# TaWeiTu/vp8

Measured on NVIDIA B200. Metric: decoded 1080p frames/s, higher is better.
Workload: dtype u8

## Files before the change

vp8_b200/csrc/cuda/recon_kernels.cu:

```cuda
#include "recon_kernels.h"

#include <algorithm>
#include <cstring>

namespace vp8r {

__constant__ int c_taps[2][8][2];
__constant__ int c_taps6[2][8][6];
__constant__ unsigned short c_bpred_lut[10 * 16];

static int PackTaps(int a, int b, int c, int d) {
  return (a & 0xff) | ((b & 0xff) << 8) | ((c & 0xff) << 16) | ((d & 0xff) << 24);
}

static void BuildBpredLut(unsigned short *lut) {
  auto L = [](int k) { return 3 - k; };
  auto A = [](int k) { return 5 + k; };
  const int P = 4;
  auto put3 = [&](int mode, int y, int x, int a, int b, int c) {
    lut[mode * 16 + y * 4 + x] = (unsigned short)(a | (b << 4) | (c << 8) | (0 << 12));
  };
  auto put2 = [&](int mode, int y, int x, int a, int c) {
    lut[mode * 16 + y * 4 + x] = (unsigned short)(a | (a << 4) | (c << 8) | (1 << 12));
  };
// ... 347 lines not shown
      out1 = AddResidual4(out1, rb.x, rb.y);
    }
    uint8_t *d = job.cur.y + (ptrdiff_t)(mb_r * 16 + y0) * job.pitch_y + mb_c * 16 + 4 * w;
    *reinterpret_cast<unsigned *>(d) = out0;
    *reinterpret_cast<unsigned *>(d + job.pitch_y) = out1;
  }
  {
    const int pl = lane >> 4, y = (lane >> 1) & 7, w = lane & 1;
    const unsigned *h = s.hc[pl];
    unsigned out;
    if (cfr) {
      unsigned e[6], o[6];
#pragma unroll
      for (int k = 0; k < 6; ++k) {
        const unsigned r = h[(y + k) * 2 + w];
        e[k] = __byte_perm(r, 0, 0x4240);
        o[k] = __byte_perm(r, 0, 0x4341);
      }
      out = Vert6(e, o, c_taps6[bil][cfr]);
    } else if (cfc == 0) {
      const int dx2 = ((g.cwx + kBorder) & 15) + 2;
      const unsigned *p = reinterpret_cast<const unsigned *>((pl ? tile->cv : tile->cu) + (y + 2) * kTmaChromaBoxW) + (dx2 >> 2) + w;
      out = __funnelshift_r(p[0], p[1], (dx2 & 3) * 8);
    } else {
      out = h[(y + 2) * 2 + w];
    }
    if (has_res) {
      const uint2 ra = *reinterpret_cast<const uint2 *>(&s.res[16 + pl * 4 + (y >> 2) * 2 + w][(y & 3) * 4]);
      out = AddResidual4(out, ra.x, ra.y);
    }
    uint8_t *d = (pl ? job.cur.v : job.cur.u) + (ptrdiff_t)(mb_r * 8 + y) * job.pitch_c + mb_c * 8 + 4 * w;
    *reinterpret_cast<unsigned *>(d) = out;
  }
}

constexpr int kInterWarps = 4;
constexpr int kInterMinBlocks = 14;

__device__ __forceinline__ void InterOneMacroblock(const DevFrameJob &job, int mb_r, int mb_c, int lane, InterScratch &scratch, InterTile *tile) {
  const int mb_index = mb_r * job.mb_cols + mb_c;
  vp8r_mb_info mb;
  {
    const int4 *p = reinterpret_cast<const int4 *>(job.mbs + mb_index);
    int4 a = __ldg(p), b = __ldg(p + 1);
    mb.flags = a.x; mb.coef_mask = a.y; mb.coef_offset = a.z;
    mb.mv[0] = (short)(a.w & 0xffff); mb.mv[1] = (short)(a.w >> 16);
    mb.aux[0] = b.x; mb.aux[1] = b.y;
  }
  if (!(mb.flags & VP8R_MB_IS_INTER)) return;

  const bool split = ((mb.flags >> VP8R_MB_MODE_SHIFT) & 7) == 4;
  WholeMbGeometry geo{};
  if (!split) {
    geo = WholeGeometry(job, mb, mb_r, mb_c);
    if (lane == 0) {
      const DevTensorMap *maps = job.ref_tmap[(mb.flags >> VP8R_MB_REF_SHIFT) & 3];
      MbarExpectTx(&tile->bar, kInterTileTxBytes);
      TmaLoad2D(tile->luma, maps + 0, (geo.wx + kBorder) & ~15, geo.wy + kBorder, &tile->bar);
      TmaLoad2D(tile->cu, maps + 1, (geo.cwx + kBorder) & ~15, geo.cwy + kBorder, &tile->bar);
      TmaLoad2D(tile->cv, maps + 2, (geo.cwx + kBorder) & ~15, geo.cwy + kBorder, &tile->bar);
    }
  }
  const bool has_res = mb.coef_mask != 0;
  if (has_res) WarpResidual(job, mb, lane, scratch);
  if (!split) {
    InterMacroblockWhole(job, mb_r, mb_c, lane, scratch, has_res, geo, tile);
    return;
  }
  __syncwarp();
  if (lane >= 24) return;

  const int ref_id = (mb.flags >> VP8R_MB_REF_SHIFT) & 3;
  const int *split_mv = reinterpret_cast<const int *>(job.payload + (size_t)mb.aux[0] * 16);

  int mvr, mvc, bx, by, pitch, plane_w, plane_h;
  const uint8_t *ref;
  uint8_t *dst;
  if (lane < 16) {
    const int m = __ldg(split_mv + lane);
    mvr = (short)(m & 0xffff);
    mvc = m >> 16;
    by = mb_r * 16 + (lane >> 2) * 4;
    bx = mb_c * 16 + (lane & 3) * 4;
    pitch = job.pitch_y;
    plane_w = job.mb_cols * 16;
    plane_h = job.mb_rows * 16;
    ref = job.ref[ref_id].y;
    dst = job.cur.y;
  } else {
    const int b = lane & 3, i = b >> 1, j = b & 1;
    const int k0 = i * 8 + j * 2;
    const int m0 = __ldg(split_mv + k0), m1 = __ldg(split_mv + k0 + 1), m2 = __ldg(split_mv + k0 + 4),
              m3 = __ldg(split_mv + k0 + 5);
    const int sr = s16((short)(m0 & 0xffff) + (short)(m1 & 0xffff) + (short)(m2 & 0xffff) + (short)(m3 & 0xffff));
    const int sc = s16((m0 >> 16) + (m1 >> 16) + (m2 >> 16) + (m3 >> 16));
    mvr = (sr >= 0 ? (sr + 4) : (sr - 4)) / 8;
    mvc = (sc >= 0 ? (sc + 4) : (sc - 4)) / 8;
    if (job.version == 3) {
      mvr &= ~7;
      mvc &= ~7;
    }
    by = mb_r * 8 + i * 4;
    bx = mb_c * 8 + j * 4;
    pitch = job.pitch_c;
    plane_w = job.mb_cols * 8;
    plane_h = job.mb_rows * 8;
    ref = lane < 20 ? job.ref[ref_id].u : job.ref[ref_id].v;
    dst = lane < 20 ? job.cur.u : job.cur.v;
  }

  const int fr = mvr & 7, fc = mvc & 7;
  int wy = by + (mvr >> 3) - 2, wx = bx + (mvc >> 3) - 2;
  wy = min(max(wy, -kBorder), plane_h + kBorder - 9);
  wx = min(max(wx, -kBorder), plane_w + kBorder - 9);
  const uint8_t *__restrict__ wp = ref + (ptrdiff_t)wy * pitch + wx;
  const uint2 *__restrict__ wrow = reinterpret_cast<const uint2 *>(wp - ((size_t)wp & 7));
  const bool upper = ((size_t)wp & 4) != 0;
  const unsigned shift = ((unsigned)(size_t)wp & 3u) * 8;
  const int wpitch = pitch >> 3;

  const int bil = job.version != 0;
  const int r_lo = fr ? 0 : 2, r_hi = fr ? 9 : 6;
  const int t03 = c_taps[bil][fc][0], t45 = c_taps[bil][fc][1];
  const TapsAt ta = MakeTapsAt(t03, t45);
  unsigned h[9];
#pragma unroll
  for (int i = 0; i < 9; ++i) {
    if (i >= r_lo && i < r_hi) {
      const uint2 a = __ldg(wrow + i * wpitch), b = __ldg(wrow + i * wpitch + 1);
      const unsigned w0 = upper ? a.y : a.x, w1 = upper ? b.x : a.y, w2 = upper ? b.y : b.x;
      const unsigned lo = __funnelshift_r(w0, w1, shift), mid = __funnelshift_r(w1, w2, shift), hi = w2 >> shift;
      h[i] = fc ? Filter4T(lo, mid, hi, t03, t45, ta) : __funnelshift_r(lo, mid, 16);
    }
  }
  unsigned out[4];
  if (fr) {
    const int v03 = c_taps[bil][fr][0], v45 = c_taps[bil][fr][1];
    const int t[6] = {(signed char)v03, (signed char)(v03 >> 8), (signed char)(v03 >> 16), v03 >> 24,
                      (signed char)v45, (signed char)(v45 >> 8)};
    unsigned e[9], o[9];
#pragma unroll
    for (int k = 0; k < 9; ++k) {
      e[k] = __byte_perm(h[k], 0, 0x4240);
      o[k] = __byte_perm(h[k], 0, 0x4341);
    }
#pragma unroll
    for (int i = 0; i < 4; ++i) out[i] = Vert6(e + i, o + i, t);
  } else {
#pragma unroll
    for (int i = 0; i < 4; ++i) out[i] = h[2 + i];
  }
  uint8_t *d = dst + (ptrdiff_t)by * pitch + bx;
  const uint2 *rp = reinterpret_cast<const uint2 *>(scratch.res[lane]);
#pragma unroll
  for (int i = 0; i < 4; ++i) {
    unsigned v = out[i];
    if (has_res) {
      const uint2 r = rp[i];
      v = AddResidual4(v, r.x, r.y);
    }
    *reinterpret_cast<unsigned *>(d + (ptrdiff_t)i * pitch) = v;
  }
}

__global__ void __launch_bounds__(kInterWarps * 32, kInterMinBlocks) InterKernel(const DevFrameJob *__restrict__ jobs) {
  __shared__ InterScratch s_scratch[kInterWarps];
  __shared__ InterTile s_tile[kInterWarps];
  const DevFrameJob &job = jobs[blockIdx.z];
  const int warp = __shfl_sync(0xffffffffu, (int)(threadIdx.x >> 5), 0), lane = threadIdx.x & 31;
  const int mb_r = blockIdx.y, cols = job.mb_cols;
  const int mb_c = blockIdx.x * kInterWarps + warp;
  if (mb_r >= job.mb_rows || mb_c >= cols) return;
  if (JobFailed(job) || JobInter(job) == 0) return;
  if (lane == 0) MbarInit(&s_tile[warp].bar, 1);
  __syncwarp();
  InterOneMacroblock(job, mb_r, mb_c, lane, s_scratch[warp], &s_tile[warp]);
  __syncwarp();
}

cudaError_t LaunchInter(const DevFrameJob *jobs, int n_frames, int max_cols, int max_rows, cudaStream_t st) {
  if (max_rows > 65535 || n_frames > 65535) return cudaErrorInvalidValue;
  dim3 grid((max_cols + kInterWarps - 1) / kInterWarps, max_rows, n_frames);
  InterKernel<<<grid, kInterWarps * 32, 0, st>>>(jobs);
  return cudaGetLastError();
}

constexpr int kWaveWarps = 32;

__device__ __forceinline__ void WaitRow(volatile int *progress, int row, int need) {
  if (row < 0) return;
  while (progress[row] < need) __nanosleep(40);
  __threadfence_block();
}
__device__ __forceinline__ void PublishRow(volatile int *progress, int row, int done, int lane) {
  __syncwarp();
  __threadfence_block();
  if (lane == 0) progress[row] = done;
}

struct __align__(16) IntraScratch {
  short y2[16];
  short res[24][16];
  unsigned char tile[17][24];
  unsigned char order[24];
};

__device__ __forceinline__ void PredictMbBlock(const DevFrameJob &job, int mb_r, int mb_c, int lane, int ymode,
                                               int uvmode, bool do_luma, const short *res, bool has_res) {
  const bool luma = lane < 16;
  const int n4 = luma ? 4 : 2;
  const int first = luma ? 0 : (lane < 20 ? 16 : 20);
  const int b = lane - first, i = luma ? (b >> 2) : (b >> 1), j = luma ? (b & 3) : (b & 1);
  const int pitch = luma ? job.pitch_y : job.pitch_c;
  uint8_t *plane = luma ? job.cur.y : (lane < 20 ? job.cur.u : job.cur.v);
  const int n = luma ? 16 : 8;
  uint8_t *mbp = plane + (ptrdiff_t)(mb_r * n) * pitch + mb_c * n;
  const bool active = lane < 24 && (do_luma || !luma);
  const int mode = luma ? ymode : uvmode;
  const bool have_above = mb_r > 0, have_left = mb_c > 0;

  unsigned aw = 0x7f7f7f7fu;
  int l[4] = {129, 129, 129, 129};
  int P = have_above ? (have_left ? 0 : 129) : 127;
  if (lane < 24) {
    if (have_above) aw = *reinterpret_cast<const unsigned *>(mbp - pitch + 4 * j);
    if (have_left) {
#pragma unroll
      for (int k = 0; k < 4; ++k) l[k] = mbp[(ptrdiff_t)(4 * i + k) * pitch - 1];
    }
    if (have_above && have_left) P = mbp[-pitch - 1];
  }
  int sum_a = (int)__dp4a(aw, 0x01010101u, 0u);
  int sum_l = l[0] + l[1] + l[2] + l[3];
  int tot_a = 0, tot_l = 0;
#pragma unroll
  for (int k = 0; k < 4; ++k) {
    int va = __shfl_sync(0xffffffffu, sum_a, first + (k < n4 ? k : 0));
    int vl = __shfl_sync(0xffffffffu, sum_l, first + (k < n4 ? k * n4 : 0));
    if (k < n4) {
      tot_a += va;
      tot_l += vl;
    }
  }
  if (!active) return;

  unsigned rows[4];
  if (mode == 1) {
    rows[0] = rows[1] = rows[2] = rows[3] = aw;
  } else if (mode == 2) {
#pragma unroll
    for (int k = 0; k < 4; ++k) rows[k] = (unsigned)l[k] * 0x01010101u;
  } else if (mode == 0) {
    int v = 128;
    if (have_above || have_left) {
      int shf = (luma ? 3 : 2) + (have_above ? 1 : 0) + (have_left ? 1 : 0);
      int sum = (have_above ? tot_a : 0) + (have_left ? tot_l : 0);
      v = (sum + (1 << (shf - 1))) >> shf;
    }
    rows[0] = rows[1] = rows[2] = rows[3] = (unsigned)v * 0x01010101u;
  } else {
#pragma unroll
    for (int k = 0; k < 4; ++k) {
      unsigned o = 0;
#pragma unroll
      for (int x = 0; x < 4; ++x) o |= (unsigned)clamp255(l[k] + (int)((aw >> (8 * x)) & 0xff) - P) << (8 * x);
      rows[k] = o;
    }
  }
  uint8_t *d = mbp + (ptrdiff_t)(4 * i) * pitch + 4 * j;
#pragma unroll
  for (int k = 0; k < 4; ++k) {
    unsigned v = rows[k];
    if (has_res) {
      unsigned o = 0;
#pragma unroll
      for (int x = 0; x < 4; ++x) o |= (unsigned)clamp255(s16((int)((v >> (8 * x)) & 0xff) + res[k * 4 + x])) << (8 * x);
      v = o;
    }
    *reinterpret_cast<unsigned *>(d + (ptrdiff_t)k * pitch) = v;
  }
}

__device__ __forceinline__ void PredictBpred(const DevFrameJob &job, int mb_r, int mb_c, int lane,
                                             const vp8r_mb_info &mb, IntraScratch &s, unsigned res_mask,
                                             const unsigned short *lut) {
  const int pitch = job.pitch_y;
  uint8_t *mbp = job.cur.y + (ptrdiff_t)(mb_r * 16) * pitch + mb_c * 16;
  if (lane < 21) {
    int col = lane - 1, v;
    if (mb_r == 0) {
      v = 127;
    } else if (col < 0) {
      v = mb_c == 0 ? 129 : mbp[-pitch - 1];
    } else if (col >= 16 && mb_c + 1 == job.mb_cols) {
      v = mbp[-pitch + 15];
    } else {
      v = mbp[-pitch + col];
    }
    s.tile[0][4 + col] = (unsigned char)v;
  }
  if (lane < 16) s.tile[1 + lane][3] = (unsigned char)(mb_c == 0 ? 129 : mbp[(ptrdiff_t)lane * pitch - 1]);
  __syncwarp();

  const int py = (lane >> 2) & 3, px = lane & 3;
  for (int b = 0; b < 16; ++b) {
    const int i = b >> 2, j = b & 3;
    const int mode = (int)((mb.aux[b >> 3] >> ((b & 7) * 4)) & 15);
    int E = 0;
    if (lane < 4) {
      E = s.tile[1 + 4 * i + (3 - lane)][3 + 4 * j];
    } else if (lane < 9) {
      E = s.tile[4 * i][3 + 4 * j + (lane - 4)];
    } else if (lane < 13) {
      const int row = (j == 3) ? 0 : 4 * i;
      E = s.tile[row][3 + 4 * j + (lane - 4)];
    }
    const unsigned e = lut[mode * 16 + (lane & 15)];
    const int x0 = __shfl_sync(0xffffffffu, E, e & 15);
    const int x1 = __shfl_sync(0xffffffffu, E, (e >> 4) & 15);
    const int x2 = __shfl_sync(0xffffffffu, E, (e >> 8) & 15);
    const int dc_in = (lane < 4 || (lane >= 5 && lane < 9)) ? E : 0;
    const int dc = (__reduce_add_sync(0xffffffffu, dc_in) + 4) >> 3;
    const int kind = e >> 12;
    int v;
    if (kind == 0) v = (x0 + 2 * x1 + x2 + 2) >> 2;
    else if (kind == 1) v = (x0 + x2 + 1) >> 1;
    else if (kind == 2) v = dc;
    else v = clamp255(x0 + x1 - x2);
    if (lane < 16) {
      if ((res_mask >> b) & 1) v = clamp255(s16(v + s.res[b][lane]));
      s.tile[1 + 4 * i + py][4 + 4 * j + px] = (unsigned char)v;
    }
    __syncwarp();
  }
  if (lane < 16) {
    const unsigned *t = reinterpret_cast<const unsigned *>(&s.tile[1 + lane][4]);
    uint4 v = make_uint4(t[0], t[1], t[2], t[3]);
    *reinterpret_cast<uint4 *>(mbp + (ptrdiff_t)lane * pitch) = v;
  }
}

__device__ __forceinline__ void IntraMacroblock(const DevFrameJob &job, int r, int c, int lane, IntraScratch &s,
                                                const unsigned short *lut, volatile int *progress) {
  vp8r_mb_info mb;
  {
    const int4 *p = reinterpret_cast<const int4 *>(job.mbs + r * job.mb_cols + c);
    int4 a = __ldg(p), b = __ldg(p + 1);
    a.x = __shfl_sync(0xffffffffu, a.x, 0); a.y = __shfl_sync(0xffffffffu, a.y, 0);
    a.z = __shfl_sync(0xffffffffu, a.z, 0); a.w = __shfl_sync(0xffffffffu, a.w, 0);
    b.x = __shfl_sync(0xffffffffu, b.x, 0); b.y = __shfl_sync(0xffffffffu, b.y, 0);
    mb.flags = a.x; mb.coef_mask = a.y; mb.coef_offset = a.z;
    mb.aux[0] = b.x; mb.aux[1] = b.y;
  }
  const bool has_res = mb.coef_mask != 0;
  if (has_res) WarpResidual(job, mb, lane, s);
  if (progress) WaitRow(progress, r - 1, min(c + 2, job.mb_cols));
  __syncwarp();
  const int ymode = (mb.flags >> VP8R_MB_MODE_SHIFT) & 7, uvmode = (mb.flags >> VP8R_MB_UVMODE_SHIFT) & 3;
  PredictMbBlock(job, r, c, lane, ymode, uvmode, ymode != 4, lane < 24 ? s.res[lane] : s.res[0], has_res);
  if (ymode == 4) PredictBpred(job, r, c, lane, mb, s, mb.coef_mask >> 1, lut);
}

__global__ void __launch_bounds__(kWaveWarps * 32) IntraKernel(const DevFrameJob *__restrict__ jobs) {
  extern __shared__ __align__(16) unsigned char smem_raw[];
  const DevFrameJob &job = jobs[blockIdx.x];
  if (JobFailed(job) || JobIntra(job) == 0 || JobIntraLevels(job) != 0) return;
  const int rows = job.mb_rows, cols = job.mb_cols;
  volatile int *progress = reinterpret_cast<volatile int *>(smem_raw);
  unsigned short *lut = reinterpret_cast<unsigned short *>(smem_raw + ((rows * 4 + 15) & ~15));
  IntraScratch *scratch = reinterpret_cast<IntraScratch *>(reinterpret_cast<unsigned char *>(lut) + 320);
  for (int i = threadIdx.x; i < rows; i += blockDim.x) progress[i] = 0;
  for (int i = threadIdx.x; i < 160; i += blockDim.x) lut[i] = c_bpred_lut[i];
  __syncthreads();

  const int warp = __shfl_sync(0xffffffffu, (int)(threadIdx.x >> 5), 0), lane = threadIdx.x & 31;
  IntraScratch &s = scratch[warp];
  for (int r = warp; r < rows; r += kWaveWarps) {
    for (int c0 = 0; c0 < cols; c0 += 32) {
      unsigned flags = 0;
      if (c0 + lane < cols) flags = __ldg(&job.mbs[r * cols + c0 + lane].flags);
      unsigned intra_mask = __ballot_sync(0xffffffffu, (c0 + lane < cols) && !(flags & VP8R_MB_IS_INTER));
      while (intra_mask) {
        const int k = __ffs(intra_mask) - 1;
        intra_mask &= intra_mask - 1;
        const int c = c0 + k;
        IntraMacroblock(job, r, c, lane, s, lut, progress);
        PublishRow(progress, r, c + 1, lane);
      }
      PublishRow(progress, r, min(c0 + 32, cols), lane);
    }
  }
}

constexpr int kFlatWarps = 8;
__global__ void __launch_bounds__(kFlatWarps * 32, 8) IntraFlatKernel(const DevFrameJob *__restrict__ jobs, int level) {
  __shared__ __align__(16) unsigned short lut[160];
  __shared__ IntraScratch scratch[kFlatWarps];
  const DevFrameJob &job = jobs[blockIdx.y];
  if (JobFailed(job) || job.dyn || level >= job.n_intra_levels) return;
  const unsigned first = __ldg(job.intra_levels + level), end = __ldg(job.intra_levels + level + 1);
  if (first + blockIdx.x * kFlatWarps >= end) return;
  for (int i = threadIdx.x; i < 160; i += blockDim.x) lut[i] = c_bpred_lut[i];
  __syncthreads();
  const int warp = __shfl_sync(0xffffffffu, (int)(threadIdx.x >> 5), 0), lane = threadIdx.x & 31;
  const unsigned slot = first + blockIdx.x * kFlatWarps + warp;
  if (slot >= end) return;
  const unsigned mb_index = __ldg(job.intra_levels + job.n_intra_levels + 1 + slot);
  const int r = mb_index / job.mb_cols, c = mb_index - r * job.mb_cols;
  IntraMacroblock(job, r, c, lane, scratch[warp], lut, nullptr);
}

constexpr int kLevelWarps = 16;
__global__ void __launch_bounds__(kLevelWarps * 32) IntraLevelsKernel(const DevFrameJob *__restrict__ jobs) {
  __shared__ __align__(16) unsigned short lut[160];
  __shared__ IntraScratch scratch[kLevelWarps];
  const DevFrameJob &job = jobs[blockIdx.x];
  if (JobFailed(job) || !job.dyn) return;
  const int n_levels = JobIntraLevels(job);
  if (n_levels == 0) return;
  for (int i = threadIdx.x; i < 160; i += blockDim.x) lut[i] = c_bpred_lut[i];
  __syncthreads();
  const int warp = __shfl_sync(0xffffffffu, (int)(threadIdx.x >> 5), 0), lane = threadIdx.x & 31;
  const uint32_t *tab = JobLevelTable(job);
  const uint32_t *order = tab + n_levels + 1;
  for (int level = 0; level < n_levels; ++level) {
    const unsigned first = tab[level], end = tab[level + 1];
    for (unsigned slot = first + warp; slot < end; slot += kLevelWarps) {
      const unsigned mb_index = order[slot];
      const int r = mb_index / job.mb_cols, c = mb_index - r * job.mb_cols;
      IntraMacroblock(job, r, c, lane, scratch[warp], lut, nullptr);
    }
    __syncthreads();
  }
}

cudaError_t LaunchIntraLevels(const DevFrameJob *jobs, int n_frames, cudaStream_t st) {
  IntraLevelsKernel<<<n_frames, kLevelWarps * 32, 0, st>>>(jobs);
  return cudaGetLastError();
}

cudaError_t LaunchIntraFlat(const DevFrameJob *jobs, int n_frames, int level, int max_count, cudaStream_t st) {
  if (max_count <= 0) return cudaSuccess;
  dim3 grid((max_count + kFlatWarps - 1) / kFlatWarps, n_frames);
  IntraFlatKernel<<<grid, kFlatWarps * 32, 0, st>>>(jobs, level);
  return cudaGetLastError();
}

static size_t IntraSmemBytes(int max_rows) {
  return ((size_t(max_rows) * 4 + 15) & ~size_t(15)) + 320 + sizeof(IntraScratch) * kWaveWarps;
}

cudaError_t LaunchIntra(const DevFrameJob *jobs, int n_frames, int max_rows, cudaStream_t st) {
  size_t smem = IntraSmemBytes(max_rows);
  static size_t configured[64] = {};
  int dev = 0;
  cudaGetDevice(&dev);
  size_t &mark = configured[dev & 63];
  if (smem > 48 * 1024 && smem > mark) {
    cudaError_t e = cudaFuncSetAttribute(IntraKernel, cudaFuncAttributeMaxDynamicSharedMemorySize, (int)smem);
    if (e != cudaSuccess) return e;
    mark = smem;
  }
  IntraKernel<<<n_frames, kWaveWarps * 32, smem, st>>>(jobs);
  return cudaGetLastError();
}

struct LfLimits {
  int interior, hev, edge_mb, edge_sb;
};

__device__ __forceinline__ LfLimits MakeLimits(int level, int sharp, bool key) {
  LfLimits l;
  int in = level;
  if (sharp) {
    in >>= (sharp > 4) ? 2 : 1;
    in = min(in, 9 - sharp);
  }
  l.interior = max(in, 1);
  if (key) l.hev = level >= 40 ? 2 : (level >= 15 ? 1 : 0);
  else l.hev = level >= 40 ? 3 : (level >= 20 ? 2 : (level >= 15 ? 1 : 0));
  l.edge_mb = (level + 2) * 2 + l.interior;
  l.edge_sb = level * 2 + l.interior;
  return l;
}

__device__ __forceinline__ int AddClamp255(int p, int d) { return min(max(p + d, 0), 255); }

template <bool kMbEdge>
__device__ __forceinline__ void LfEdge(int *v, const LfLimits &lim, bool simple) {
  const int edge = kMbEdge ? lim.edge_mb : lim.edge_sb;
  const int p3 = v[0], p2 = v[1], p1 = v[2], p0 = v[3], q0 = v[4], q1 = v[5], q2 = v[6], q3 = v[7];
  const int d_p1q1 = p1 - q1, d_q0p0 = q0 - p0;
  const bool edge_ok = abs(d_q0p0) * 2 + (abs(d_p1q1) >> 1) <= edge;
  const int s = clamp128(d_p1q1);
  if (simple) {
    const int a = clamp128(s + 3 * d_q0p0);
    const int f1 = min(a + 4, 127) >> 3, f2 = min(a + 3, 127) >> 3;
    v[3] = AddClamp255(p0, edge_ok ? f2 : 0);
    v[4] = AddClamp255(q0, edge_ok ? -f1 : 0);
    return;
  }
  const int a_p1p0 = abs(p1 - p0), a_q1q0 = abs(q1 - q0);
  const int interior = max(max(max(abs(p3 - p2), abs(p2 - p1)), a_p1p0), max(max(a_q1q0, abs(q1 - q2)), abs(q2 - q3)));
  const bool on = edge_ok && interior <= lim.interior;
  const bool hev = max(a_p1p0, a_q1q0) > lim.hev;
  if (kMbEdge) {
    const int w = clamp128(s + 3 * d_q0p0);
    const int f1 = min(w + 4, 127) >> 3, f2 = min(w + 3, 127) >> 3;
    const int a27 = (27 * w + 63) >> 7, a18 = (18 * w + 63) >> 7, a9 = (9 * w + 63) >> 7;
    const int dp0 = on ? (hev ? f2 : a27) : 0, dq0 = on ? (hev ? f1 : a27) : 0;
    const int d1 = (on && !hev) ? a18 : 0, d2 = (on && !hev) ? a9 : 0;
    v[1] = AddClamp255(p2, d2);
    v[2] = AddClamp255(p1, d1);
    v[3] = AddClamp255(p0, dp0);
    v[4] = AddClamp255(q0, -dq0);
    v[5] = AddClamp255(q1, -d1);
    v[6] = AddClamp255(q2, -d2);
  } else {
    const int a = clamp128((hev ? s : 0) + 3 * d_q0p0);
    const int f1 = min(a + 4, 127) >> 3, f2 = min(a + 3, 127) >> 3;
    const int a2 = (on && !hev) ? ((f1 + 1) >> 1) : 0;
    v[2] = AddClamp255(p1, a2);
    v[3] = AddClamp255(p0, on ? f2 : 0);
    v[4] = AddClamp255(q0, on ? -f1 : 0);
    v[5] = AddClamp255(q1, -a2);
  }
}

__global__ void __launch_bounds__(256) BorderKernel(const DevFrameJob *__restrict__ jobs) {
  const DevFrameJob &job = jobs[blockIdx.y];
  for (int pl = 0; pl < 3; ++pl) {
    uint8_t *base = pl == 0 ? job.cur.y : (pl == 1 ? job.cur.u : job.cur.v);
    const int pitch = pl == 0 ? job.pitch_y : job.pitch_c;
    const int w = job.mb_cols * (pl == 0 ? 16 : 8), h = job.mb_rows * (pl == 0 ? 16 : 8);
    const int side_items = h * 8;
    const int vecs = (w + 2 * kBorder) / 8;
    const int total = side_items + vecs * 2 * kBorder;
    for (int t = blockIdx.x * blockDim.x + threadIdx.x; t < total; t += gridDim.x * blockDim.x) {
      if (t < side_items) {
        const int row = t >> 3, part = t & 7;
        uint8_t *rowp = base + (ptrdiff_t)row * pitch;
        const unsigned v = (part < 4 ? rowp[0] : rowp[w - 1]) * 0x01010101u;
        uint8_t *d = part < 4 ? rowp - kBorder + 8 * part : rowp + w + 8 * (part - 4);
        *reinterpret_cast<uint2 *>(d) = make_uint2(v, v);
      } else {
        const int u = t - side_items;
        const int k = u / vecs, x8 = (u - k * vecs) * 8 - kBorder;
        const int src_row = k < kBorder ? 0 : h - 1;
        const int dst_row = k < kBorder ? k - kBorder : h + (k - kBorder);
        const uint8_t *srow = base + (ptrdiff_t)src_row * pitch;
        uint2 v;
        if (x8 < 0) {
          const unsigned e = srow[0] * 0x01010101u;
          v = make_uint2(e, e);
        } else if (x8 >= w) {
          const unsigned e = srow[w - 1] * 0x01010101u;
          v = make_uint2(e, e);
        } else {
          v = *reinterpret_cast<const uint2 *>(srow + x8);
        }
        *reinterpret_cast<uint2 *>(base + (ptrdiff_t)dst_row * pitch + x8) = v;
      }
    }
  }
}

constexpr int kFiltWarps = 4;
constexpr int kMaxBands = 64;
constexpr int kBandStride = 8;
constexpr int kFiltCtasPerSm = 8;

static int SmCount() {
  static int count[64] = {};
  int dev = 0;
  cudaGetDevice(&dev);
  int &c = count[dev & 63];
  if (c == 0 && cudaDeviceGetAttribute(&c, cudaDevAttrMultiProcessorCount, dev) != cudaSuccess) c = 148;
  return c;
}

constexpr int kTilePitch = 20;
struct __align__(16) FiltTile {
  unsigned char bytes[(16 + 8 + 8) * kTilePitch];
};

__device__ __forceinline__ int LoadFlagAcquire(const int *p) {
  int v;
  asm volatile("ld.acquire.gpu.global.s32 %0, [%1];" : "=r"(v) : "l"(p) : "memory");
  return v;
}

__global__ void __launch_bounds__(kFiltWarps * 32, kFiltCtasPerSm) FilterKernel(const DevFrameJob *__restrict__ jobs, int n_frames,
                                                                   int n_bands, int *__restrict__ sync, int resident_ctas) {
  extern __shared__ __align__(16) unsigned char smem_raw[];
  __shared__ int s_ticket;
  if (threadIdx.x == 0) s_ticket = atomicAdd(&sync[0], 1);
  __syncthreads();
  const bool band_major = n_frames * n_bands > resident_ctas;
  const int band = band_major ? s_ticket / n_frames : s_ticket % n_bands;
  const int frame = band_major ? s_ticket - band * n_frames : s_ticket / n_bands;
  const DevFrameJob &job = jobs[frame];
  const int rows = job.mb_rows, cols = job.mb_cols;
  const int rpb = (rows + n_bands - 1) / n_bands;
  const int r0 = band * rpb, r1 = min(rows, r0 + rpb);
  if (job.lf_level == 0 || r0 >= r1 || JobFailed(job)) return;
  int *gflag = sync + 1 + frame * n_bands;
  volatile int *lprog = reinterpret_cast<volatile int *>(smem_raw);
  FiltTile *tiles = reinterpret_cast<FiltTile *>(smem_raw + ((rpb * 4 + 15) & ~15));
  for (int i = threadIdx.x; i < rpb; i += blockDim.x) lprog[i] = 0;
  __syncthreads();

  const int warp = __shfl_sync(0xffffffffu, (int)(threadIdx.x >> 5), 0), lane = threadIdx.x & 31;
  const bool simple = job.filter_type != 0;
  const int sharpness = job.sharpness;
  const bool key_frame = job.key_frame != 0;
  const vp8r_mb_info *const mbs = job.mbs;
  const bool luma = lane < 16;
  const int n = luma ? 16 : 8;
  const int line = luma ? lane : (lane & 7);
  uint8_t *plane = luma ? job.cur.y : (lane < 24 ? job.cur.u : job.cur.v);
  const int pitch = luma ? job.pitch_y : job.pitch_c;
  const bool lane_on = luma || !simple;
  const int n_words = n / 4;
  unsigned char *const tb = reinterpret_cast<unsigned char *>(tiles + warp);
  const int tbase = luma ? 0 : (lane < 24 ? 16 : 24) * kTilePitch;
  const int trow_off = tbase + line * kTilePitch;
  const int tcol_off = tbase + line;

  for (int lr = warp; lr < r1 - r0; lr += kFiltWarps) {
    const int r = r0 + lr;
    const bool last_of_band = (r == r1 - 1) && (band + 1 < n_bands);
    const bool has_above = r > 0;
    const bool above_local = lr > 0;
    uint8_t *rowp = plane + (ptrdiff_t)(r * n + line) * pitch;
    const uint8_t *abovep = plane + (ptrdiff_t)(r * n - 4) * pitch + line;
    const vp8r_mb_info *mbrow = mbs + (size_t)r * cols;
    unsigned nxt[4] = {0, 0, 0, 0};
    unsigned flags32 = lane < cols ? __ldg(&mbrow[lane].flags) : 0u;
    if (lane_on) {
      if (luma) {
        const uint4 t = *reinterpret_cast<const uint4 *>(rowp);
        nxt[0] = t.x; nxt[1] = t.y; nxt[2] = t.z; nxt[3] = t.w;
      } else {
        const uint2 t = *reinterpret_cast<const uint2 *>(rowp);
        nxt[0] = t.x; nxt[1] = t.y;
      }
    }
    unsigned carry = 0;
    int a4n[4] = {0, 0, 0, 0};
    int gseen = 0;
    bool have_above = false;

    for (int c = 0; c < cols; ++c) {
      unsigned cur[4] = {nxt[0], nxt[1], nxt[2], nxt[3]};
      if (c && (c & 31) == 0) flags32 = c + lane < cols ? __ldg(&mbrow[c + lane].flags) : 0u;
      const unsigned flags = __shfl_sync(0xffffffffu, flags32, c & 31);
      if (c + 1 < cols) {
        if (lane_on) {
          const uint8_t *np = rowp + (c + 1) * n;
          if (luma) {
            const uint4 t = *reinterpret_cast<const uint4 *>(np);
            nxt[0] = t.x; nxt[1] = t.y; nxt[2] = t.z; nxt[3] = t.w;
          } else {
            const uint2 t = *reinterpret_cast<const uint2 *>(np);
            nxt[0] = t.x; nxt[1] = t.y;
          }
// ... 546 lines not shown
```

Before: 82520.

## Predict two B_PRED subblocks per warp step along anti-diagonal wavefront

The 4x4 B_PRED loop used to predict the 16 subblocks one after another, with only 16 of the 32 lanes doing work. It now walks anti-diagonals in 10 steps, so each half-warp predicts an independent subblock at the same time. Shuffles use width 16, and the DC sum is split into two half-masked reductions. The kernel's launch bounds also gain a minimum-blocks hint of 2, which may limit registers per thread.

```diff
diff --git a/vp8_b200/csrc/cuda/recon_kernels.cu b/vp8_b200/csrc/cuda/recon_kernels.cu
--- a/vp8_b200/csrc/cuda/recon_kernels.cu
+++ b/vp8_b200/csrc/cuda/recon_kernels.cu
@@ -673,34 +673,41 @@
   if (lane < 16) s.tile[1 + lane][3] = (unsigned char)(mb_c == 0 ? 129 : mbp[(ptrdiff_t)lane * pitch - 1]);
   __syncwarp();
 
-  const int py = (lane >> 2) & 3, px = lane & 3;
-  for (int b = 0; b < 16; ++b) {
-    const int i = b >> 2, j = b & 3;
-    const int mode = (int)((mb.aux[b >> 3] >> ((b & 7) * 4)) & 15);
+  const int half = lane >> 4, sl = lane & 15;
+  const int py = sl >> 2, px = sl & 3;
+  for (int t = 0; t < 10; ++t) {
+    const int i0 = t <= 3 ? 0 : (t - 2) >> 1;
+    const int i = i0 + half, j = t - 2 * i;
+    const bool on = i < 4 && j >= 0;
+    const int b = on ? 4 * i + j : 0;
+    const int bi = b >> 2, bj = b & 3;
+    const int mode = (int)((((b & 8) ? mb.aux[1] : mb.aux[0]) >> ((b & 7) * 4)) & 15);
     int E = 0;
-    if (lane < 4) {
-      E = s.tile[1 + 4 * i + (3 - lane)][3 + 4 * j];
-    } else if (lane < 9) {
-      E = s.tile[4 * i][3 + 4 * j + (lane - 4)];
-    } else if (lane < 13) {
-      const int row = (j == 3) ? 0 : 4 * i;
-      E = s.tile[row][3 + 4 * j + (lane - 4)];
-    }
-    const unsigned e = lut[mode * 16 + (lane & 15)];
-    const int x0 = __shfl_sync(0xffffffffu, E, e & 15);
-    const int x1 = __shfl_sync(0xffffffffu, E, (e >> 4) & 15);
-    const int x2 = __shfl_sync(0xffffffffu, E, (e >> 8) & 15);
-    const int dc_in = (lane < 4 || (lane >= 5 && lane < 9)) ? E : 0;
-    const int dc = (__reduce_add_sync(0xffffffffu, dc_in) + 4) >> 3;
+    if (sl < 4) {
+      E = s.tile[1 + 4 * bi + (3 - sl)][3 + 4 * bj];
+    } else if (sl < 9) {
+      E = s.tile[4 * bi][3 + 4 * bj + (sl - 4)];
+    } else if (sl < 13) {
+      const int row = (bj == 3) ? 0 : 4 * bi;
+      E = s.tile[row][3 + 4 * bj + (sl - 4)];
+    }
+    const unsigned e = lut[mode * 16 + sl];
+    const int x0 = __shfl_sync(0xffffffffu, E, e & 15, 16);
+    const int x1 = __shfl_sync(0xffffffffu, E, (e >> 4) & 15, 16);
+    const int x2 = __shfl_sync(0xffffffffu, E, (e >> 8) & 15, 16);
+    const int dc_in = (sl < 4 || (sl >= 5 && sl < 9)) ? E : 0;
+    const int dc_lo = __reduce_add_sync(0xffffffffu, half ? 0 : dc_in);
+    const int dc_hi = __reduce_add_sync(0xffffffffu, half ? dc_in : 0);
+    const int dc = ((half ? dc_hi : dc_lo) + 4) >> 3;
     const int kind = e >> 12;
     int v;
     if (kind == 0) v = (x0 + 2 * x1 + x2 + 2) >> 2;
     else if (kind == 1) v = (x0 + x2 + 1) >> 1;
     else if (kind == 2) v = dc;
     else v = clamp255(x0 + x1 - x2);
-    if (lane < 16) {
-      if ((res_mask >> b) & 1) v = clamp255(s16(v + s.res[b][lane]));
-      s.tile[1 + 4 * i + py][4 + 4 * j + px] = (unsigned char)v;
+    if (on) {
+      if ((res_mask >> b) & 1) v = clamp255(s16(v + s.res[b][sl]));
+      s.tile[1 + 4 * bi + py][4 + 4 * bj + px] = (unsigned char)v;
     }
     __syncwarp();
   }
@@ -732,7 +739,7 @@
   if (ymode == 4) PredictBpred(job, r, c, lane, mb, s, mb.coef_mask >> 1, lut);
 }
 
-__global__ void __launch_bounds__(kWaveWarps * 32) IntraKernel(const DevFrameJob *__restrict__ jobs) {
+__global__ void __launch_bounds__(kWaveWarps * 32, 2) IntraKernel(const DevFrameJob *__restrict__ jobs) {
   extern __shared__ __align__(16) unsigned char smem_raw[];
   const DevFrameJob &job = jobs[blockIdx.x];
   if (JobFailed(job) || JobIntra(job) == 0 || JobIntraLevels(job) != 0) return;
```

After: 82680 (median of 6 runs). About the same (+0.2%).
